# sideprotocol/plonky2-gpu

Hardware: AMD Instinct MI355X
Metric: NTTs/sec at 2^20 Goldilocks (higher is better)
Workload: dtype u64 (Goldilocks, integer modular)

## Files before the change

plonky2_gpu_amd/csrc/ntt_direct.hip:

```cpp

#include "ntt_kernels.h"

namespace plonky2_hip {
namespace nttk {

namespace {

#ifndef NTT_TAIL_GROUPED
#define NTT_TAIL_GROUPED 1
#endif
#ifndef DIRECT_DIAG_HOOKS
#define DIRECT_TILE_BARRIER() lds_barrier()
#define DIRECT_LOAD_TILE(t) (t)
#define DIRECT_STORE_TILE(t) (t)
#define DIRECT_DIAG_TAIL_FRONT_ON 0
#define DIRECT_DIAG_SAME_STORES_ON 0
#define DIRECT_NT_LOAD_COL false
#define DIRECT_NT_STORE_COL false
#define DIRECT_NT_LOAD_ROW false
#define DIRECT_NT_STORE_ROW false
#define DIRECT_TOUCH_STATE
#define DIRECT_TOUCH_COL(t_in_a)
#define DIRECT_TOUCH_ROW(t_in_a)
#endif

__device__ __forceinline__ uint64_t lds_ld(const unsigned char *lds, uint32_t off) { return *reinterpret_cast<const uint64_t *>(lds + off); }
__device__ __forceinline__ void lds_st(unsigned char *lds, uint32_t off, uint64_t v) { *reinterpret_cast<uint64_t *>(lds + off) = v; }
template <bool NT = false>
__device__ __forceinline__ uint64_t g_ld(const uint64_t *base, uint32_t byte_off) {
    const uint64_t *q = reinterpret_cast<const uint64_t *>(reinterpret_cast<const unsigned char *>(base) + byte_off);
    if constexpr (NT) return __builtin_nontemporal_load(q);
    return *q;
}
template <bool NT = false>
__device__ __forceinline__ void g_st(uint64_t *base, uint32_t byte_off, uint64_t v) {
    uint64_t *q = reinterpret_cast<uint64_t *>(reinterpret_cast<unsigned char *>(base) + byte_off);
    if constexpr (NT)
        __builtin_nontemporal_store(v, q);
    else
        *q = v;
}
constexpr bool NT_LOAD_COL = DIRECT_NT_LOAD_COL, NT_STORE_COL = DIRECT_NT_STORE_COL, NT_LOAD_ROW = DIRECT_NT_LOAD_ROW, NT_STORE_ROW = DIRECT_NT_STORE_ROW;

template <int LOGG>
struct ColGeom {
    static constexpr int G = 1 << LOGG, LOGC = 6 - LOGG, C = 1 << LOGC, LOGR = 8 + LOGG, R = 1 << LOGR;
    static constexpr uint32_t ROWB = C * 8;
    static constexpr uint32_t SA = 16 * ROWB + (G >= 4 ? ROWB : 0);
    static constexpr uint32_t XBYTES = 16 * G * SA;
    static constexpr uint32_t TWBYTES = 16 * G * 16 * 8;
    static constexpr uint32_t LDS_BYTES = XBYTES + TWBYTES;
    static constexpr uint32_t cu_entries(uint32_t gz) { return gz * (G > 1 ? G * 16 : 256); }
    static constexpr uint32_t t2z_entries(uint32_t gz) { return G > 1 ? gz * 16 * G : 0; }
    static constexpr uint32_t cs_entries(uint32_t gz) { return gz * C; }
    static constexpr uint32_t coset_bytes(uint32_t gz) { return (cu_entries(gz) + t2z_entries(gz) + cs_entries(gz)) * 8; }
};

static_assert(ColGeom<3>::LDS_BYTES <= 160 * 1024 && ColGeom<2>::LDS_BYTES <= 160 * 1024, "the exchange image and the tables must fit the 160 KiB of LDS of a gfx950 CU");

template <int LOGG, bool NATURAL, bool COSET = false, bool FINAL = false, bool REVIN = false>
__global__ __launch_bounds__(1024) __attribute__((amdgpu_waves_per_eu(4, 4))) void ntt_col_direct_kernel(const PassParams p, const uint32_t gx, const uint32_t gy, const uint32_t gz, const uint32_t per_b) {
    using GEO = ColGeom<LOGG>;
    constexpr int G = GEO::G, LOGC = GEO::LOGC, C = GEO::C, LOGR = GEO::LOGR;
    constexpr uint32_t ROWB = GEO::ROWB, SA = GEO::SA;
    extern __shared__ __attribute__((aligned(16))) unsigned char ldsb[];
    unsigned char *X = ldsb;
    unsigned char *TW = ldsb + GEO::XBYTES;
    unsigned char *CU = TW + GEO::TWBYTES, *T2Z = CU + GEO::cu_entries(gz) * 8, *CS = T2Z + GEO::t2z_entries(gz) * 8;

    const uint32_t tid = threadIdx.x, lane = tid & 63;
    const uint32_t wave = __builtin_amdgcn_readfirstlane(tid >> 6);
    const uint32_t g = lane >> LOGC, c = lane & (C - 1);

    const uint32_t W = gridDim.x;
    const uint32_t u = (W & 7) == 0 ? (blockIdx.x & 7) * (W >> 3) + (blockIdx.x >> 3) : blockIdx.x;
    const uint32_t P = gy * gz;
    uint32_t b0, bstep, p0, pstep;
    if (per_b) {
        if constexpr (COSET) b0 = u / per_b, p0 = u % per_b;
        else b0 = u % gx, p0 = u / gx;
        bstep = gx, pstep = per_b;
    } else {
        b0 = u, bstep = W, p0 = 0, pstep = 1;
    }
    const uint32_t np_local = p0 < P ? (P - p0 + pstep - 1) / pstep : 0;
    const uint32_t nb_local = b0 < gx ? (gx - b0 + bstep - 1) / bstep : 0;
    const uint32_t n_tiles = np_local * nb_local;
    if (n_tiles == 0) return;

    for (uint32_t e = tid; e < 16u * G * 16u; e += 1024) {
        const uint32_t w_ = e / (16 * G), g_ = (e / 16) % G, ka = e % 16;
        reinterpret_cast<uint64_t *>(TW)[e] = p.twh[(ka * (16 * g_ + w_)) << (12 - LOGR)];
    }
    uint64_t t2[G > 1 ? G : 1];
    if constexpr (!COSET)
        static_for<1, G>([&](auto K_) {
            constexpr int kb = decltype(K_)::value;
            t2[kb] = p.twh[(kb * wave) << (12 - 4 - LOGG)];
        });
    if constexpr (COSET) {
        auto cs_pow = [&](uint32_t z, uint64_t ex) { return gl::mul(p.cs_hi[z * p.cs_hi_len + (uint32_t)(ex >> 10)], p.cs_lo[z * 1024 + (uint32_t)(ex & 1023)]); };
        for (uint32_t e = tid; e < GEO::cu_entries(gz); e += 1024) {
            const uint32_t i = e & 15, mid = G > 1 ? 16 * ((e >> 4) % G) : (e >> 4) & 15, z = G > 1 ? e / (16 * G) : e >> 8;
            reinterpret_cast<uint64_t *>(CU)[e] = cs_pow(z, (uint64_t)p.in_m * (((uint32_t)i << (LOGR - 4)) + mid));
        }
        for (uint32_t e = tid; e < GEO::t2z_entries(gz); e += 1024) {
            const uint32_t kb = e % G, w_ = (e / G) & 15, z = e / (16 * G);
            reinterpret_cast<uint64_t *>(T2Z)[e] = gl::mul(p.twh[(kb * w_) << (12 - 4 - LOGG)], cs_pow(z, (uint64_t)p.in_m * w_));
        }
        for (uint32_t e = tid; e < GEO::cs_entries(gz); e += 1024)
            reinterpret_cast<uint64_t *>(CS)[e] = cs_pow(e / C, (uint64_t)b0 * C + (e % C));
    }

    const uint32_t tw_base = (wave * G + g) * 128;
    const uint32_t lane_x = wave * ROWB + c * 8;
    const uint32_t pw_base = 16 * g * SA + lane_x;
    const uint32_t pr_base = g * SA + lane_x;
    constexpr bool natural = NATURAL;
    auto opaque_lane = [&]() {
        uint32_t l = lane;
        asm volatile("" : "+v"(l));
        return l;
    };
    auto kab_of = [&](uint32_t l) { return G * wave + (l >> LOGC); };
    auto xr_base_of = [&](uint32_t l) { return kab_of(l) * SA + (l & (C - 1)) * 8; };
    auto ld_off_of = [&](uint32_t l) { return (uint32_t)(((l & (C - 1)) + (uint64_t)(16 * (l >> LOGC) + wave) * p.in_m) * 8); };
    const uint64_t out_c = p.out_c ? p.out_c : 1;
    auto st_off_of = [&](uint32_t l) {
        const uint32_t kab = kab_of(l);
        const uint32_t out_row_lane = natural ? kab : (brev_rt(kab & 15, 4) << (LOGR - 4)) | (brev_rt(kab >> 4, LOGG) << 4);
        return (uint32_t)(((l & (C - 1)) * out_c + (uint64_t)out_row_lane * p.out_m) * 8);
    };

    auto tile_of = [&](uint32_t t, uint32_t &b, uint32_t &a, uint32_t &z) {
        const uint32_t bi = t / np_local, pi = t - bi * np_local;
        b = b0 + bi * bstep;
        const uint32_t pp = p0 + pi * pstep;
        if constexpr (COSET) a = pp / gz, z = pp % gz;
        else a = pp % gy, z = pp / gy;
        if (p.sweep_down) a = gy - 1 - a;
    };

    uint64_t A[16];
    const uint32_t ld_step = (uint32_t)(((uint64_t)p.in_m << (LOGR - 4)) * 8);
    auto issue_loads = [&](uint32_t t) {
        uint32_t b, a, z;
        tile_of(DIRECT_LOAD_TILE(t), b, a, z);
        if constexpr (REVIN) {
            static_assert(!COSET && NATURAL, "the reversed-input pass is the first pass of a natural-order inverse transform");
            const uint64_t *base = p.src + (a * p.in_sa + z * p.in_sz);
            const uint32_t l = opaque_lane();
            const uint32_t L = b * C + (l & (C - 1)), m0 = 16 * (l >> LOGC) + wave;
            const uint32_t cols = (uint32_t)p.in_m;
            uint32_t off = L ? (((uint32_t)GEO::R - 1 - m0) * cols + (cols - L)) * 8 : (((uint32_t)GEO::R - m0) * cols) * 8;
            const bool wraps = L == 0 && m0 == 0;
            static_for<0, 16>([&](auto I_) {
                constexpr int i = decltype(I_)::value;
                if constexpr (i == 0) A[i] = g_ld<NT_LOAD_COL>(base, wraps ? 0u : off);
                else A[i] = g_ld<NT_LOAD_COL>(base, off);
                if constexpr (i < 15) off -= ld_step;
            });
            return;
        }
        const uint64_t *base = p.src + (a * p.in_sa + b * p.in_sb + z * p.in_sz);
        uint32_t off = ld_off_of(opaque_lane());
        static_for<0, 16>([&](auto I_) {
            constexpr int i = decltype(I_)::value;
            A[i] = g_ld<NT_LOAD_COL>(base, off);
            if constexpr (i < 15) off += ld_step;
        });
    };

    uint64_t B[16];
    uint64_t cc0 = 1, cstep = 1;
    constexpr bool kept_twiddles = !COSET && !FINAL;
    uint64_t cw[kept_twiddles ? 8 : 1], cstep8 = 1;
    uint32_t chain_b = 0xFFFFFFFFu;
    const uint32_t st_row = (uint32_t)(p.out_m * 8);

    uint64_t cc = 1;
    uint64_t *obase = p.dst;
    uint32_t so = 0;
    auto tail_begin = [&](uint32_t k) {
        uint32_t b, a, z;
        tile_of(k, b, a, z);
        if (!FINAL && b != chain_b) {
            chain_b = b;
            const uint32_t l = opaque_lane();
            const uint64_t L = (uint64_t)b * C + (l & (C - 1));
            cc0 = wpow(p, L * kab_of(l));
            if (p.chain_scale != 1) cc0 = gl::mul(cc0, p.chain_scale);
            cstep = wpow(p, L << (4 + LOGG));
            asm volatile("" : "+v"(cc0), "+v"(cstep));
            if constexpr (kept_twiddles) {
                cw[0] = cc0;
                static_for<1, 8>([&](auto J_) {
                    constexpr int j = decltype(J_)::value;
                    cw[j] = gl::mul(cw[j - 1], cstep);
                });
                const uint64_t s2 = gl::mul(cstep, cstep), s4 = gl::mul(s2, s2);
                cstep8 = gl::mul(s4, s4);
            }
        }
        if constexpr (DIRECT_DIAG_SAME_STORES_ON) tile_of(0, b, a, z);
        obase = p.dst + (a * p.out_sa + b * p.out_sb + (COSET ? brev_rt(z, p.rate_bits) : z) * p.out_sz);
        if constexpr (COSET) cc = gl::mul(cc0, lds_ld(CS, (z * C + (opaque_lane() & (C - 1))) * 8));
        else cc = cc0;
        so = st_off_of(opaque_lane());
    };
    auto tail_unit = [&](auto J_) {
        constexpr int j = decltype(J_)::value;
        constexpr int s3 = brev_c(j, 4);
        if constexpr (FINAL) {
            B[s3] = gl::canon(B[s3]);
        } else if constexpr (kept_twiddles) {
            if constexpr (j < 8) B[s3] = gl::mul(B[s3], cw[j]);
            else B[s3] = gl::mul(B[s3], gl::mul(cw[j - 8], cstep8));
        } else {
            B[s3] = gl::mul(B[s3], cc);
            if constexpr (j < 15) cc = gl::mul(cc, cstep);
        }
        const uint32_t row = natural ? (uint32_t)(j << (4 + LOGG)) : (uint32_t)s3;
        g_st<NT_STORE_COL>(obase, so + row * st_row, B[s3]);
        __builtin_amdgcn_sched_barrier(0);
    };
    auto tail_store = [&](auto J_) {
        constexpr int j = decltype(J_)::value;
        constexpr int s3 = brev_c(j, 4);
        const uint32_t row = natural ? (uint32_t)(j << (4 + LOGG)) : (uint32_t)s3;
        g_st<NT_STORE_COL>(obase, so + row * st_row, B[s3]);
        __builtin_amdgcn_sched_barrier(0);
    };
    auto tail_units = [&](auto LO_, auto HI_) {
        constexpr int LO = decltype(LO_)::value, HI = decltype(HI_)::value, N = HI - LO;
        if constexpr (NTT_TAIL_GROUPED && kept_twiddles && N >= 1 && N <= 8) {
            uint64_t tw[N];
            constexpr int N_HI = HI > 8 ? HI - (LO > 8 ? LO : 8) : 0;
            if constexpr (N_HI > 0)
                rare_group<N_HI>([&](auto I_, gl::rare_mask &f) { constexpr int j = (LO > 8 ? LO : 8) + decltype(I_)::value; tw[j - LO] = gl::mul_f(cw[j - 8], cstep8, f); },
                                 [&](auto I_, gl::rare_mask f) { constexpr int j = (LO > 8 ? LO : 8) + decltype(I_)::value; tw[j - LO] = gl::mul_fix(tw[j - LO], f); });
            rare_group<N>(
                [&](auto I_, gl::rare_mask &f) {
                    constexpr int j = LO + decltype(I_)::value, s3 = brev_c(j, 4);
                    if constexpr (j < 8) B[s3] = gl::mul_f(B[s3], cw[j], f);
                    else B[s3] = gl::mul_f(B[s3], tw[j - LO], f);
                },
                [&](auto I_, gl::rare_mask f) {
                    constexpr int s3 = brev_c(LO + decltype(I_)::value, 4);
                    B[s3] = gl::mul_fix(B[s3], f);
                });
            static_for<LO, HI>([&](auto J_) { tail_store(J_); });
        } else {
            static_for<LO, HI>([&](auto J_) { tail_unit(J_); });
        }
    };

    DIRECT_TOUCH_STATE
    auto first_rounds = [&](auto WITH_TAIL_, uint32_t t_in_a) {
        constexpr bool with_tail = decltype(WITH_TAIL_)::value;
        uint32_t zc = 0;
        if constexpr (COSET) {
            uint32_t b_, a_;
            tile_of(t_in_a, b_, a_, zc);
        }
        if constexpr (with_tail && DIRECT_DIAG_TAIL_FRONT_ON) tail_units(std::integral_constant<int, 0>{}, std::integral_constant<int, 16>{});
#define TAIL(lo, hi) do { if constexpr (with_tail && !DIRECT_DIAG_TAIL_FRONT_ON) tail_units(std::integral_constant<int, lo>{}, std::integral_constant<int, hi>{}); } while (0)
        TAIL(0, 4);
        if constexpr (COSET) {
            const uint32_t cu_base = (G > 1 ? (zc * G + (opaque_lane() >> LOGC)) * 16 : (zc * 16 + wave) * 16) * 8;
            mul_run<0, 16>(A, [](auto I_) { return decltype(I_)::value; }, [&](auto I_) { return lds_ld(CU, cu_base + decltype(I_)::value * 8); }, [](auto) {});
        }
        radix_dif_stage<4, 0, 3>(A);
        DIRECT_TOUCH_COL(t_in_a);
        TAIL(4, 6);
        radix_dif_stage<4, 0, 2>(A);
        TAIL(6, 8);
        radix_dif_stage<4, 0, 1>(A);
        TAIL(8, 10);
        radix_dif_stage<4, 0, 0>(A);
        TAIL(10, 12);
        mul_run<1, 16>(A, [](auto S_) { return decltype(S_)::value; }, [&](auto S_) { return lds_ld(TW, tw_base + brev_c(decltype(S_)::value, 4) * 8); },
                       [&](auto S_) {
                           constexpr int s = decltype(S_)::value;
                           if constexpr (s == 5) TAIL(12, 13);
                           if constexpr (s == 10) TAIL(13, 14);
                       });
        if constexpr (G > 1) {
            static_for<0, 16>([&](auto S_) {
                constexpr int s = decltype(S_)::value;
                constexpr int ka = brev_c(s, 4);
                lds_st(X, pw_base + ka * SA, A[s]);
            });
            tile_sync<64>();
            static_for<0, 16 / G>([&](auto J_) {
                constexpr int j = decltype(J_)::value;
                static_for<0, G>([&](auto GG_) {
                    constexpr int gg = decltype(GG_)::value;
                    A[j * G + gg] = lds_ld(X, pr_base + (16 * gg + G * j) * SA);
                });
            });
            tile_sync<64>();
            radix_dif_blocks<LOGG>(A);
            TAIL(14, 15);
            if constexpr (COSET)
                mul_run<0, 16>(A, [](auto E_) { return decltype(E_)::value; },
                               [&](auto E_) { return lds_ld(T2Z, ((zc * 16 + wave) * G + brev_c(decltype(E_)::value % G, LOGG)) * 8); }, [](auto) {});
            else
                mul_run<0, (G - 1) * (16 / G)>(A, [](auto K_) { return (decltype(K_)::value / (G - 1)) * G + 1 + decltype(K_)::value % (G - 1); },
                                               [&](auto K_) { return t2[brev_c(1 + decltype(K_)::value % (G - 1), LOGG)]; }, [](auto) {});
            static_for<0, 16 / G>([&](auto J_) {
                constexpr int j = decltype(J_)::value;
                static_for<0, G>([&](auto S_) {
                    constexpr int s2 = decltype(S_)::value;
                    constexpr int kb = brev_c(s2, LOGG);
                    lds_st(X, pr_base + (G * j + 16 * kb) * SA, A[j * G + s2]);
                });
            });
            TAIL(15, 16);
        } else {
            TAIL(14, 16);
            static_for<0, 16>([&](auto S_) {
                constexpr int s = decltype(S_)::value;
                constexpr int ka = brev_c(s, 4);
                lds_st(X, pr_base + ka * SA, A[s]);
            });
        }
#undef TAIL
    };

    lds_barrier();
    issue_loads(0);
    const uint32_t last = n_tiles - 1;
    first_rounds(std::false_type{}, 0);
    if (last > 0) issue_loads(1);
#pragma unroll 1
    for (uint32_t k = 0; k <= last; k++) {
        DIRECT_TILE_BARRIER();
        const uint32_t xr_base = xr_base_of(opaque_lane());
        static_for<0, 16>([&](auto WR_) {
            constexpr int wr = decltype(WR_)::value;
            B[wr] = lds_ld(X, xr_base + wr * ROWB);
        });
        DIRECT_TILE_BARRIER();
        radix_dif<4, 0>(B);
        tail_begin(k);
        if (k < last) {
            first_rounds(std::true_type{}, k + 1);
            if (k + 1 < last) issue_loads(k + 2);
        } else {
            tail_units(std::integral_constant<int, 0>{}, std::integral_constant<int, 16>{});
        }
    }
}

template <int LOGG, bool NATURAL, bool COSET = false, bool FINAL = false, bool REVIN = false>
hipError_t launch_col_direct_t(const PassParams &p, dim3 grid, hipStream_t stream) {
    using GEO = ColGeom<LOGG>;
    const uint32_t lds_bytes = GEO::LDS_BYTES + (COSET ? GEO::coset_bytes(grid.z) : 0);
    static DynamicLds attr;
    if (hipError_t e = allow_dynamic_lds(attr, reinterpret_cast<const void *>(&ntt_col_direct_kernel<LOGG, NATURAL, COSET, FINAL, REVIN>), lds_bytes); e != hipSuccess) return e;
    int dev = 0, cus = 256;
    if (hipGetDevice(&dev) == hipSuccess) (void)hipDeviceGetAttribute(&cus, hipDeviceAttributeMultiprocessorCount, dev);
    const uint64_t pairs = (uint64_t)grid.y * grid.z, total = pairs * grid.x;
    if (total == 0) return hipSuccess;
    if (total > 0xFFFFFFFFull) return hipErrorInvalidValue;
    uint32_t per_b = 0, wgs;
    if (grid.x <= (uint32_t)cus) {
        per_b = (uint32_t)cus / grid.x;
        if (per_b > pairs) per_b = (uint32_t)pairs;
        wgs = grid.x * per_b;
    } else {
        wgs = (uint32_t)cus;
    }
    if (COSET && per_b == 0) return hipErrorInvalidValue;
    hipLaunchKernelGGL((ntt_col_direct_kernel<LOGG, NATURAL, COSET, FINAL, REVIN>), dim3(wgs), dim3(1024), lds_bytes, stream, p, (uint32_t)grid.x, (uint32_t)grid.y, (uint32_t)grid.z, per_b);
    return hipGetLastError();
}


struct RowGeom {
    static constexpr uint32_t SQ = 136, SB = 544, SA = 8736;
    static constexpr uint32_t XBYTES = 16 * SA;
    static constexpr uint32_t TW1_STRIDE = 136, TW1_BYTES = 64 * TW1_STRIDE;
    static constexpr uint32_t TW2_STRIDE = 136, TW2_BYTES = 4 * TW2_STRIDE;
    static constexpr uint32_t LDS_BYTES = XBYTES + TW1_BYTES;
};

template <bool INVERSE>
__global__ __launch_bounds__(1024) __attribute__((amdgpu_waves_per_eu(4, 4))) void ntt_row_natural_direct_kernel(const PassParams p, const uint32_t gx, const uint32_t gy, const uint32_t gz) {
    using GEO = RowGeom;
    constexpr uint32_t SQ = GEO::SQ, SB = GEO::SB, SA = GEO::SA;
    extern __shared__ __attribute__((aligned(16))) unsigned char ldsb[];
    unsigned char *X = ldsb;
    unsigned char *TW1 = ldsb + GEO::XBYTES;

    const uint32_t tid = threadIdx.x, lane = tid & 63;
    const uint32_t wave = __builtin_amdgcn_readfirstlane(tid >> 6);

    const uint32_t W = gridDim.x;
    const uint32_t u = (W & 7) == 0 ? (blockIdx.x & 7) * (W >> 3) + (blockIdx.x >> 3) : blockIdx.x;
    const uint32_t total = gx * gy * gz;
    if (u >= total) return;
    const uint32_t n_tiles = (total - u + W - 1) / W;

    for (uint32_t e = tid; e < 64 * 16; e += 1024) {
        const uint32_t l = e >> 4, ka = e & 15;
        *reinterpret_cast<uint64_t *>(TW1 + l * GEO::TW1_STRIDE + ka * 8) = p.twh[(ka * l) << 2];
    }

    const uint32_t q = lane & 3, hi4 = lane >> 2;
    const uint32_t tw1_base = lane * GEO::TW1_STRIDE;
    const uint32_t pw_base = hi4 * SB + q * SQ + wave * 8;
    const uint32_t pr_base = hi4 * SA + q * SQ + wave * 8;
    auto opaque_lane = [&]() {
        uint32_t l = lane;
        asm volatile("" : "+v"(l));
        return l;
    };

    auto tile_of = [&](uint32_t t, uint32_t &b, uint32_t &a, uint32_t &z) {
        const uint32_t id = u + t * W;
        b = id % gx;
        const uint32_t r = id / gx;
        a = r % gy;
        z = r / gy;
        if (p.sweep_down) a = gy - 1 - a;
    };

    uint64_t A[16];
    auto issue_loads = [&](uint32_t t) {
        uint32_t b, a, z;
        tile_of(DIRECT_LOAD_TILE(t), b, a, z);
        const uint32_t row = (b * 16 + wave + p.row_shift) & (p.t_limit - 1);
        const uint64_t *base = p.src + (a * p.in_sa + z * p.in_sz + (uint64_t)row * p.in_t);
        const uint32_t off = opaque_lane() * 8;
        static_for<0, 16>([&](auto I_) {
            constexpr int i = decltype(I_)::value;
            A[i] = g_ld<NT_LOAD_ROW>(base, off + i * 512);
        });
    };

    uint64_t B[16];
    const uint32_t kbhi = wave >> 2, kalo = wave & 3;
    uint64_t *obase = p.dst;
    uint32_t o_lane = 0;
    const uint32_t n_mask = (1u << p.log_n) - 1;
    auto tail_begin = [&](uint32_t k) {
        uint32_t b, a, z;
        tile_of(DIRECT_STORE_TILE(k), b, a, z);
        obase = p.dst + (a * p.out_sa + z * p.out_sz);
        const uint32_t l = opaque_lane();
        const uint32_t r = l & 15, ka = 4 * (l >> 4) + kalo;
        const uint32_t k1 = (b * 16 + r + p.row_shift) & (p.t_limit - 1);
        o_lane = k1 + (uint32_t)p.out_m * (ka + 64 * kbhi);
    };
    auto tail_unit = [&](auto J_) {
        constexpr int s = decltype(J_)::value;
        constexpr int kblo = s >> 2, kc = brev_c(s & 3, 2);
// ... 212 lines not shown
            const uint32_t kbhi = l & 3, base = (l >> 2) * 32 + kbhi * 2048;
            static_for<0, 16>([&](auto R_) {
                constexpr int r = decltype(R_)::value;
                B[r] = lds_ld(X, base + (r >> 2) * 512 + (((uint32_t)(r & 3) ^ kbhi) * 8));
            });
        }
        tile_sync<64>();
        radix_dif_blocks<2>(B);
        {
            const uint32_t l = opaque_lane();
            const uint32_t ka = l >> 2, kbhi = l & 3;
            const uint32_t pa = brev_rt(ka, 4), sw = pa >> 2;
            const uint32_t base = (pa * 64 + brev_rt(kbhi, 2) * 4) * 8;
            static_for<0, 16>([&](auto R_) {
                constexpr int r = decltype(R_)::value;
                constexpr uint32_t kblo = r >> 2, s2 = r & 3;
                lds_st(X, base + brev_c(kblo, 2) * 128 + ((s2 ^ sw) * 8), gl::canon(B[r]));
            });
        }
        tile_sync<64>();
        {
            const uint32_t l = opaque_lane();
            uint64_t *obase = p.dst + row_ptr(k, true);
            static_for<0, 16>([&](auto R_) {
                constexpr int r = decltype(R_)::value;
                const uint32_t slot = r * 64 + (l & ~3u) + ((l & 3) ^ (uint32_t)(r >> 2));
                const uint64_t v = lds_ld(X, slot * 8);
                g_st(obase, l * 8 + r * 512, v);
            });
        }
        tile_sync<64>();
        __builtin_amdgcn_sched_barrier(0);
        if (more) issue_loads_other_half(k + 1);
        __builtin_amdgcn_sched_barrier(0);
    };

    lds_barrier();
    if (n_rows == 0) return;
    issue_loads(0);
    issue_loads_other_half(0);
    first_round();
    if (n_rows > 1) issue_loads(1);
#pragma unroll 1
    for (uint32_t k = 0; k < n_rows; k++) {
        rest_of_row(k, k + 1 < n_rows);
        if (k + 1 < n_rows) {
            first_round();
            if (k + 2 < n_rows) issue_loads(k + 2);
        }
    }
}

template <bool HALVES = false>
hipError_t launch_row_inplace_direct_t(const PassParams &p, dim3 grid, hipStream_t stream) {
    constexpr uint32_t lds_bytes = HALVES ? RowInplaceGeom::LDS_BYTES_HALVES : RowInplaceGeom::LDS_BYTES;
    static DynamicLds attr;
    if (hipError_t e = allow_dynamic_lds(attr, reinterpret_cast<const void *>(&ntt_row_inplace_direct_kernel<HALVES>), lds_bytes); e != hipSuccess) return e;
    int dev = 0, cus = 256;
    if (hipGetDevice(&dev) == hipSuccess) (void)hipDeviceGetAttribute(&cus, hipDeviceAttributeMultiprocessorCount, dev);
    const uint64_t rows_total = (uint64_t)p.t_limit * grid.y * grid.z * (HALVES ? 2 : 1);
    if (rows_total == 0) return hipSuccess;
    if (rows_total > 0xFFFFFFFFull) return hipErrorInvalidValue;
    const uint64_t need = (rows_total + 15) / 16;
    const uint32_t wgs = (uint32_t)(need < (uint64_t)cus ? need : (uint64_t)cus);
    hipLaunchKernelGGL(ntt_row_inplace_direct_kernel<HALVES>, dim3(wgs), dim3(1024), lds_bytes, stream, p, (uint32_t)rows_total, p.t_limit, (uint32_t)grid.y);
    return hipGetLastError();
}

}

bool col_direct_coset_ok(int logg, dim3 grid) {
    int dev = 0, cus = 256;
    if (hipGetDevice(&dev) == hipSuccess) (void)hipDeviceGetAttribute(&cus, hipDeviceAttributeMultiprocessorCount, dev);
    if (grid.x > (uint32_t)cus || grid.z == 0) return false;
    const uint32_t limit = device_lds_limit();
    switch (logg) {
        case 0: return ColGeom<0>::LDS_BYTES + ColGeom<0>::coset_bytes(grid.z) <= limit;
        case 1: return ColGeom<1>::LDS_BYTES + ColGeom<1>::coset_bytes(grid.z) <= limit;
        case 2: return ColGeom<2>::LDS_BYTES + ColGeom<2>::coset_bytes(grid.z) <= limit;
        default: return false;
    }
}

hipError_t launch_col_direct(int logg, const PassParams &p, dim3 grid, hipStream_t stream) {
    const bool nat = p.flags & F_NATURAL;
    if (p.flags & F_COSET) {
        if (nat || !col_direct_coset_ok(logg, grid)) return hipErrorInvalidValue;
        switch (logg) {
            case 0: return launch_col_direct_t<0, false, true>(p, grid, stream);
            case 1: return launch_col_direct_t<1, false, true>(p, grid, stream);
            case 2: return launch_col_direct_t<2, false, true>(p, grid, stream);
            default: return hipErrorInvalidValue;
        }
    }
    switch (logg) {
        case 0: return nat ? launch_col_direct_t<0, true>(p, grid, stream) : launch_col_direct_t<0, false>(p, grid, stream);
        case 1: return nat ? launch_col_direct_t<1, true>(p, grid, stream) : launch_col_direct_t<1, false>(p, grid, stream);
        case 2: return nat ? launch_col_direct_t<2, true>(p, grid, stream) : launch_col_direct_t<2, false>(p, grid, stream);
        case 3: return nat ? launch_col_direct_t<3, true>(p, grid, stream) : launch_col_direct_t<3, false>(p, grid, stream);
        default: return hipErrorInvalidValue;
    }
}


hipError_t launch_col_direct_reversed_input(const PassParams &p, dim3 grid, hipStream_t stream) {
    if (!(p.flags & F_NATURAL) || (p.flags & F_COSET) || p.in_t != 1 || p.in_m != (1u << 11) || p.in_sb != 8) return hipErrorInvalidValue;
    return launch_col_direct_t<3, true, false, false, true>(p, grid, stream);
}

hipError_t launch_col_direct_final(const PassParams &p, dim3 grid, hipStream_t stream) {
    if (!(p.flags & F_NATURAL) || (p.flags & F_COSET)) return hipErrorInvalidValue;
    return launch_col_direct_t<3, true, false, true>(p, grid, stream);
}

hipError_t launch_row_inplace_direct(const PassParams &p, dim3 grid, hipStream_t stream) { return launch_row_inplace_direct_t<false>(p, grid, stream); }
hipError_t launch_row_inplace_direct_2048(const PassParams &p, dim3 grid, hipStream_t stream) { return launch_row_inplace_direct_t<true>(p, grid, stream); }

hipError_t launch_row_natural_direct(const PassParams &p, dim3 grid, hipStream_t stream) {
    return (p.flags & F_INVERSE) ? launch_row_natural_direct_t<true>(p, grid, stream) : launch_row_natural_direct_t<false>(p, grid, stream);
}

}
}
```

plonky2_gpu_amd/csrc/ntt_kernels.h:

```cpp
#pragma once
#include <atomic>
#include <hip/hip_runtime.h>
#include <stdint.h>

#include <type_traits>

#include "gl_field.h"

namespace plonky2_hip {
namespace nttk {

enum : uint32_t { F_LOAD_ROWS = 1, F_STORE_ROWS = 2, F_NATURAL = 4, F_INVERSE = 8, F_COSET = 16,
                  F_WIDE = 32,
                  F_RAW_OUT = 64,
                  F_FINAL_COL = 128 };

struct PassParams {
    const uint64_t *src;
    uint64_t *dst;
    const uint64_t *twl;
    const uint64_t *twh;
    const uint64_t *cs_hi;
    const uint64_t *cs_lo;
    uint64_t in_sa, in_sb, in_sz, in_t, in_m;
// ... 192 lines not shown
    constexpr auto KQ = [](int kblo, int q) { return (39 * q * (4 * KBHI + kblo)) % 192; };
    constexpr auto NEGQ = [](int kblo, int q) { return (39 * q * (4 * KBHI + kblo)) % 192 >= 96; };
    {
        gl::rare_mask fm[12];
        static_for<0, 12>([&](auto I_) {
            constexpr int i = decltype(I_)::value, kblo = i / 3, q = 1 + i % 3, KK = KQ(kblo, q) % 96;
            v[4 * kblo + q] = gl::mul_pow2_f<KK>(v[4 * kblo + q], fm[i]);
        });
        __builtin_amdgcn_sched_barrier(RARE_FENCE_MASK);
        gl::rare_mask any = 0;
        static_for<0, 12>([&](auto I_) { any |= fm[decltype(I_)::value]; });
        if (GL_RARE_ANY(any))
            static_for<0, 12>([&](auto I_) {
                constexpr int i = decltype(I_)::value, kblo = i / 3, q = 1 + i % 3, KK = KQ(kblo, q) % 96;
                v[4 * kblo + q] = gl::mul_pow2_fix<KK>(v[4 * kblo + q], fm[i]);
            });
    }
    auto bfly = [&](auto CNEG_, auto I0_, auto I1_, gl::rare_mask &f0, gl::rare_mask &f1) {
        constexpr bool cneg = decltype(CNEG_)::value;
        constexpr int i0 = decltype(I0_)::value, i1 = decltype(I1_)::value;
        if constexpr (cneg) gl::bfly_f<false>(v[i0], v[i1], v[i1], v[i0], f1, f0);
        else gl::bfly_f<false>(v[i0], v[i1], v[i0], v[i1], f0, f1);
    };
    auto fix = [&](auto IS_SUM_, auto SHIFT_, auto I_, gl::rare_mask f, gl::rare_mask fshift) {
        constexpr bool is_sum = decltype(IS_SUM_)::value;
        constexpr int shift = decltype(SHIFT_)::value, i = decltype(I_)::value;
        if constexpr (shift == 0) {
            v[i] = is_sum ? gl::add_fix(v[i], f) : gl::sub_fix(v[i], f);
        } else {
            v[i] = gl::mul_pow2_fix<shift>(v[i], fshift);
            const uint64_t c = gl::masked_const<gl::eps_times_pow2(shift)>(f);
            v[i] = is_sum ? gl::add(v[i], c) : gl::sub(v[i], c);
        }
    };
    using std::integral_constant;
    using std::bool_constant;
    {
        gl::rare_mask f0[8], f1[8], fm[4];
        static_for<0, 4>([&](auto B_) {
            constexpr int kblo = decltype(B_)::value, b = 4 * kblo;
            bfly(bool_constant<NEGQ(kblo, 2)>{}, integral_constant<int, b>{}, integral_constant<int, b + 2>{}, f0[2 * kblo], f1[2 * kblo]);
            bfly(bool_constant<NEGQ(kblo, 1) != NEGQ(kblo, 3)>{}, integral_constant<int, b + 1>{}, integral_constant<int, b + 3>{}, f0[2 * kblo + 1], f1[2 * kblo + 1]);
        });
        static_for<0, 4>([&](auto B_) {
            constexpr int kblo = decltype(B_)::value;
            v[4 * kblo + 3] = gl::mul_pow2_f<48>(v[4 * kblo + 3], fm[kblo]);
        });
        __builtin_amdgcn_sched_barrier(RARE_FENCE_MASK);
        gl::rare_mask any = 0;
        static_for<0, 8>([&](auto I_) { any |= f0[decltype(I_)::value] | f1[decltype(I_)::value]; });
        static_for<0, 4>([&](auto I_) { any |= fm[decltype(I_)::value]; });
        if (GL_RARE_ANY(any))
            static_for<0, 4>([&](auto B_) {
                constexpr int kblo = decltype(B_)::value, b = 4 * kblo;
                constexpr bool na = NEGQ(kblo, 2), nb = NEGQ(kblo, 1) != NEGQ(kblo, 3);
                fix(bool_constant<!na>{}, integral_constant<int, 0>{}, integral_constant<int, b>{}, f0[2 * kblo], 0);
                fix(bool_constant<na>{}, integral_constant<int, 0>{}, integral_constant<int, b + 2>{}, f1[2 * kblo], 0);
                fix(bool_constant<!nb>{}, integral_constant<int, 0>{}, integral_constant<int, b + 1>{}, f0[2 * kblo + 1], 0);
                fix(bool_constant<nb>{}, integral_constant<int, 48>{}, integral_constant<int, b + 3>{}, f1[2 * kblo + 1], fm[kblo]);
            });
    }
    {
        gl::rare_mask f0[8], f1[8];
        static_for<0, 4>([&](auto B_) {
            constexpr int kblo = decltype(B_)::value, b = 4 * kblo;
            bfly(bool_constant<NEGQ(kblo, 1)>{}, integral_constant<int, b>{}, integral_constant<int, b + 1>{}, f0[2 * kblo], f1[2 * kblo]);
            bfly(bool_constant<NEGQ(kblo, 1)>{}, integral_constant<int, b + 2>{}, integral_constant<int, b + 3>{}, f0[2 * kblo + 1], f1[2 * kblo + 1]);
        });
        __builtin_amdgcn_sched_barrier(RARE_FENCE_MASK);
        gl::rare_mask any = 0;
        static_for<0, 8>([&](auto I_) { any |= f0[decltype(I_)::value] | f1[decltype(I_)::value]; });
        if (GL_RARE_ANY(any))
            static_for<0, 4>([&](auto B_) {
                constexpr int kblo = decltype(B_)::value, b = 4 * kblo;
                constexpr bool n1 = NEGQ(kblo, 1);
                fix(bool_constant<!n1>{}, integral_constant<int, 0>{}, integral_constant<int, b>{}, f0[2 * kblo], 0);
                fix(bool_constant<n1>{}, integral_constant<int, 0>{}, integral_constant<int, b + 1>{}, f1[2 * kblo], 0);
                fix(bool_constant<!n1>{}, integral_constant<int, 0>{}, integral_constant<int, b + 2>{}, f0[2 * kblo + 1], 0);
                fix(bool_constant<n1>{}, integral_constant<int, 0>{}, integral_constant<int, b + 3>{}, f1[2 * kblo + 1], 0);
            });
    }
}

template <int NT_>
__device__ __forceinline__ void tile_sync() {
    if constexpr (NT_ == 64) {
        __builtin_amdgcn_fence(__ATOMIC_ACQ_REL, "wavefront");
        __builtin_amdgcn_wave_barrier();
    } else {
        __syncthreads();
    }
}

__device__ __forceinline__ void lds_barrier() { asm volatile("s_waitcnt lgkmcnt(0)\n\ts_barrier" ::: "memory"); }


struct DynamicLds {
    std::atomic<uint8_t> set[64] = {};
};
inline uint32_t device_lds_limit() {
    int dev = 0, bytes = 0;
    if (hipGetDevice(&dev) != hipSuccess || hipDeviceGetAttribute(&bytes, hipDeviceAttributeMaxSharedMemoryPerBlock, dev) != hipSuccess || bytes <= 0)
        return 64 * 1024;
    return (uint32_t)bytes;
}
inline hipError_t allow_dynamic_lds(DynamicLds &st, const void *fn, uint32_t lds_bytes) {
    int dev = 0;
    hipError_t e = hipGetDevice(&dev);
    if (e != hipSuccess) return e;
    std::atomic<uint8_t> &slot = st.set[dev & 63];
    if (slot.load(std::memory_order_acquire)) return hipSuccess;
    const uint32_t limit = device_lds_limit();
    e = hipFuncSetAttribute(fn, hipFuncAttributeMaxDynamicSharedMemorySize, (int)(lds_bytes > limit ? lds_bytes : limit));
    if (e != hipSuccess) return e;
    slot.store(1, std::memory_order_release);
    return hipSuccess;
}

hipError_t launch_col_direct(int logg, const PassParams &p, dim3 grid, hipStream_t stream);
hipError_t launch_col_direct_reversed_input(const PassParams &p, dim3 grid, hipStream_t stream);
hipError_t launch_col_direct_final(const PassParams &p, dim3 grid, hipStream_t stream);
bool col_direct_coset_ok(int logg, dim3 grid);
hipError_t launch_row_natural_direct(const PassParams &p, dim3 grid, hipStream_t stream);
hipError_t launch_row_inplace_direct(const PassParams &p, dim3 grid, hipStream_t stream);
hipError_t launch_row_inplace_direct_2048(const PassParams &p, dim3 grid, hipStream_t stream);

}
}
```

Measured before the change: 131,800.

## Split column-pass LDS exchange into two halves and keep upper twiddles in LDS

For the LOGG=2 column pass, the exchange image is halved and written in two phases. Waves are staggered so half read the image while the other half write their second half. Eight-plus of the sixteen per-column twiddles are precomputed into an LDS region instead of being derived with an extra multiply, which cuts register pressure and per-element multiplies. It adds barriers and LDS traffic, and includes optional (default-off) shift-twiddle radix and half-load variants.

```diff
diff --git a/plonky2_gpu_amd/csrc/ntt_direct.hip b/plonky2_gpu_amd/csrc/ntt_direct.hip
--- a/plonky2_gpu_amd/csrc/ntt_direct.hip
+++ b/plonky2_gpu_amd/csrc/ntt_direct.hip
@@ -1,4 +1,5 @@
 
+#include "knobs.h"
 #include "ntt_kernels.h"
 
 namespace plonky2_hip {
@@ -8,6 +9,18 @@
 
 #ifndef NTT_TAIL_GROUPED
 #define NTT_TAIL_GROUPED 1
+#endif
+#ifndef NTT_COL_RESIDENT_TWIDDLES
+#define NTT_COL_RESIDENT_TWIDDLES 1
+#endif
+#ifndef NTT_COL_SHIFT_TWIDDLE
+#define NTT_COL_SHIFT_TWIDDLE 0
+#endif
+#ifndef NTT_COL_LOAD_HALVES
+#define NTT_COL_LOAD_HALVES 0
+#endif
+#ifndef NTT_COL_CW_REGS
+#define NTT_COL_CW_REGS 6
 #endif
 #ifndef DIRECT_DIAG_HOOKS
 #define DIRECT_TILE_BARRIER() lds_barrier()
@@ -50,6 +63,10 @@
     static constexpr uint32_t XBYTES = 16 * G * SA;
     static constexpr uint32_t TWBYTES = 16 * G * 16 * 8;
     static constexpr uint32_t LDS_BYTES = XBYTES + TWBYTES;
+    static constexpr uint32_t XBYTES_SPLIT = 8 * G * SA;
+    static constexpr int CW_REGS = NTT_COL_CW_REGS;
+    static constexpr uint32_t CW_STRIDE = 1024 * 8, CWBYTES = (16 - CW_REGS) * CW_STRIDE;
+    static constexpr uint32_t LDS_BYTES_SPLIT = XBYTES_SPLIT + TWBYTES + CWBYTES;
     static constexpr uint32_t cu_entries(uint32_t gz) { return gz * (G > 1 ? G * 16 : 256); }
     static constexpr uint32_t t2z_entries(uint32_t gz) { return G > 1 ? gz * 16 * G : 0; }
     static constexpr uint32_t cs_entries(uint32_t gz) { return gz * C; }
@@ -57,15 +74,28 @@
 };
 
 static_assert(ColGeom<3>::LDS_BYTES <= 160 * 1024 && ColGeom<2>::LDS_BYTES <= 160 * 1024, "the exchange image and the tables must fit the 160 KiB of LDS of a gfx950 CU");
-
-template <int LOGG, bool NATURAL, bool COSET = false, bool FINAL = false, bool REVIN = false>
+static_assert(ColGeom<2>::CW_REGS >= 1 && ColGeom<2>::CW_REGS <= 8, "the kept twiddles");
+static_assert(ColGeom<2>::LDS_BYTES_SPLIT == 69632 + 8192 + (16 - ColGeom<2>::CW_REGS) * 8192 && ColGeom<2>::LDS_BYTES_SPLIT <= 160 * 1024, "two-phase image, TW and the resident twiddles");
+
+template <int LOGG, bool COSET, bool FINAL, bool REVIN, bool PREVIOUS>
+struct ColForm {
+    static constexpr bool tuned = LOGG == 2 && !COSET && !FINAL && !REVIN && !PREVIOUS;
+    static constexpr bool SPLIT = tuned && NTT_COL_RESIDENT_TWIDDLES;
+    static constexpr bool SHIFT2 = tuned && NTT_COL_SHIFT_TWIDDLE;
+    static constexpr uint32_t LDS_BYTES = SPLIT ? ColGeom<LOGG>::LDS_BYTES_SPLIT : ColGeom<LOGG>::LDS_BYTES;
+};
+
+template <int LOGG, bool NATURAL, bool COSET = false, bool FINAL = false, bool REVIN = false, bool PREVIOUS = false>
 __global__ __launch_bounds__(1024) __attribute__((amdgpu_waves_per_eu(4, 4))) void ntt_col_direct_kernel(const PassParams p, const uint32_t gx, const uint32_t gy, const uint32_t gz, const uint32_t per_b) {
     using GEO = ColGeom<LOGG>;
+    using FORM = ColForm<LOGG, COSET, FINAL, REVIN, PREVIOUS>;
+    constexpr bool SPLIT = FORM::SPLIT, SHIFT2 = FORM::SHIFT2;
     constexpr int G = GEO::G, LOGC = GEO::LOGC, C = GEO::C, LOGR = GEO::LOGR;
     constexpr uint32_t ROWB = GEO::ROWB, SA = GEO::SA;
     extern __shared__ __attribute__((aligned(16))) unsigned char ldsb[];
     unsigned char *X = ldsb;
-    unsigned char *TW = ldsb + GEO::XBYTES;
+    unsigned char *TW = ldsb + (SPLIT ? GEO::XBYTES_SPLIT : GEO::XBYTES);
+    unsigned char *CW = TW + GEO::TWBYTES;
     unsigned char *CU = TW + GEO::TWBYTES, *T2Z = CU + GEO::cu_entries(gz) * 8, *CS = T2Z + GEO::t2z_entries(gz) * 8;
 
     const uint32_t tid = threadIdx.x, lane = tid & 63;
@@ -93,7 +123,7 @@
         reinterpret_cast<uint64_t *>(TW)[e] = p.twh[(ka * (16 * g_ + w_)) << (12 - LOGR)];
     }
     uint64_t t2[G > 1 ? G : 1];
-    if constexpr (!COSET)
+    if constexpr (!COSET && !SHIFT2)
         static_for<1, G>([&](auto K_) {
             constexpr int kb = decltype(K_)::value;
             t2[kb] = p.twh[(kb * wave) << (12 - 4 - LOGG)];
@@ -114,7 +144,7 @@
 
     const uint32_t tw_base = (wave * G + g) * 128;
     const uint32_t lane_x = wave * ROWB + c * 8;
-    const uint32_t pw_base = 16 * g * SA + lane_x;
+    const uint32_t pw_base = (SPLIT ? 8 : 16) * g * SA + lane_x;
     const uint32_t pr_base = g * SA + lane_x;
     constexpr bool natural = NATURAL;
     auto opaque_lane = [&]() {
@@ -123,7 +153,7 @@
         return l;
     };
     auto kab_of = [&](uint32_t l) { return G * wave + (l >> LOGC); };
-    auto xr_base_of = [&](uint32_t l) { return kab_of(l) * SA + (l & (C - 1)) * 8; };
+    auto xr_base_of = [&](uint32_t l) { return (SPLIT ? kab_of(l) & (8 * G - 1) : kab_of(l)) * SA + (l & (C - 1)) * 8; };
     auto ld_off_of = [&](uint32_t l) { return (uint32_t)(((l & (C - 1)) + (uint64_t)(16 * (l >> LOGC) + wave) * p.in_m) * 8); };
     const uint64_t out_c = p.out_c ? p.out_c : 1;
     auto st_off_of = [&](uint32_t l) {
@@ -143,10 +173,12 @@
 
     uint64_t A[16];
     const uint32_t ld_step = (uint32_t)(((uint64_t)p.in_m << (LOGR - 4)) * 8);
-    auto issue_loads = [&](uint32_t t) {
+    auto issue_loads_part = [&](uint32_t t, auto LO_, auto HI_) {
+        constexpr int LO = decltype(LO_)::value, HI = decltype(HI_)::value;
         uint32_t b, a, z;
         tile_of(DIRECT_LOAD_TILE(t), b, a, z);
         if constexpr (REVIN) {
+            static_assert(LO == 0 && HI == 16, "the reversed-input pass loads whole tiles");
             static_assert(!COSET && NATURAL, "the reversed-input pass is the first pass of a natural-order inverse transform");
             const uint64_t *base = p.src + (a * p.in_sa + z * p.in_sz);
             const uint32_t l = opaque_lane();
@@ -163,18 +195,22 @@
             return;
         }
         const uint64_t *base = p.src + (a * p.in_sa + b * p.in_sb + z * p.in_sz);
-        uint32_t off = ld_off_of(opaque_lane());
-        static_for<0, 16>([&](auto I_) {
+        uint32_t off = ld_off_of(opaque_lane()) + LO * ld_step;
+        static_for<LO, HI>([&](auto I_) {
             constexpr int i = decltype(I_)::value;
             A[i] = g_ld<NT_LOAD_COL>(base, off);
-            if constexpr (i < 15) off += ld_step;
-        });
-    };
+            if constexpr (i < HI - 1) off += ld_step;
+        });
+    };
+    auto issue_loads = [&](uint32_t t) { issue_loads_part(t, std::integral_constant<int, 0>{}, std::integral_constant<int, 16>{}); };
+    uint64_t N[16];
 
     uint64_t B[16];
     uint64_t cc0 = 1, cstep = 1;
     constexpr bool kept_twiddles = !COSET && !FINAL;
-    uint64_t cw[kept_twiddles ? 8 : 1], cstep8 = 1;
+    constexpr int KEPT = SPLIT ? GEO::CW_REGS : 8;
+    uint64_t cw[kept_twiddles ? KEPT : 1], cstep8 = 1;
+    auto cw_off = [&](int j) { return (wave * 64 + opaque_lane()) * 8 + (uint32_t)(j - KEPT) * GEO::CW_STRIDE; };
     uint32_t chain_b = 0xFFFFFFFFu;
     const uint32_t st_row = (uint32_t)(p.out_m * 8);
 
@@ -194,12 +230,20 @@
             asm volatile("" : "+v"(cc0), "+v"(cstep));
             if constexpr (kept_twiddles) {
                 cw[0] = cc0;
-                static_for<1, 8>([&](auto J_) {
+                static_for<1, KEPT>([&](auto J_) {
                     constexpr int j = decltype(J_)::value;
                     cw[j] = gl::mul(cw[j - 1], cstep);
                 });
-                const uint64_t s2 = gl::mul(cstep, cstep), s4 = gl::mul(s2, s2);
-                cstep8 = gl::mul(s4, s4);
+                if constexpr (SPLIT) {
+                    uint64_t t = cw[KEPT - 1];
+                    static_for<KEPT, 16>([&](auto J_) {
+                        t = gl::mul(t, cstep);
+                        lds_st(CW, cw_off(decltype(J_)::value), t);
+                    });
+                } else {
+                    const uint64_t s2 = gl::mul(cstep, cstep), s4 = gl::mul(s2, s2);
+                    cstep8 = gl::mul(s4, s4);
+                }
             }
         }
         if constexpr (DIRECT_DIAG_SAME_STORES_ON) tile_of(0, b, a, z);
@@ -214,7 +258,8 @@
         if constexpr (FINAL) {
             B[s3] = gl::canon(B[s3]);
         } else if constexpr (kept_twiddles) {
-            if constexpr (j < 8) B[s3] = gl::mul(B[s3], cw[j]);
+            if constexpr (j < KEPT) B[s3] = gl::mul(B[s3], cw[j]);
+            else if constexpr (SPLIT) B[s3] = gl::mul(B[s3], lds_ld(CW, cw_off(j)));
             else B[s3] = gl::mul(B[s3], gl::mul(cw[j - 8], cstep8));
         } else {
             B[s3] = gl::mul(B[s3], cc);
@@ -235,14 +280,16 @@
         constexpr int LO = decltype(LO_)::value, HI = decltype(HI_)::value, N = HI - LO;
         if constexpr (NTT_TAIL_GROUPED && kept_twiddles && N >= 1 && N <= 8) {
             uint64_t tw[N];
-            constexpr int N_HI = HI > 8 ? HI - (LO > 8 ? LO : 8) : 0;
-            if constexpr (N_HI > 0)
+            constexpr int N_HI = HI > KEPT ? HI - (LO > KEPT ? LO : KEPT) : 0;
+            if constexpr (N_HI > 0 && SPLIT)
+                static_for<(LO > KEPT ? LO : KEPT), HI>([&](auto J_) { constexpr int j = decltype(J_)::value; tw[j - LO] = lds_ld(CW, cw_off(j)); });
+            else if constexpr (N_HI > 0)
                 rare_group<N_HI>([&](auto I_, gl::rare_mask &f) { constexpr int j = (LO > 8 ? LO : 8) + decltype(I_)::value; tw[j - LO] = gl::mul_f(cw[j - 8], cstep8, f); },
                                  [&](auto I_, gl::rare_mask f) { constexpr int j = (LO > 8 ? LO : 8) + decltype(I_)::value; tw[j - LO] = gl::mul_fix(tw[j - LO], f); });
             rare_group<N>(
                 [&](auto I_, gl::rare_mask &f) {
                     constexpr int j = LO + decltype(I_)::value, s3 = brev_c(j, 4);
-                    if constexpr (j < 8) B[s3] = gl::mul_f(B[s3], cw[j], f);
+                    if constexpr (j < KEPT) B[s3] = gl::mul_f(B[s3], cw[j], f);
                     else B[s3] = gl::mul_f(B[s3], tw[j - LO], f);
                 },
                 [&](auto I_, gl::rare_mask f) {
@@ -285,7 +332,39 @@
                            if constexpr (s == 5) TAIL(12, 13);
                            if constexpr (s == 10) TAIL(13, 14);
                        });
-        if constexpr (G > 1) {
+        if constexpr (SPLIT) {
+            static_for<0, 2>([&](auto H_) {
+                constexpr int h = decltype(H_)::value;
+                static_for<0, 16>([&](auto S_) {
+                    constexpr int s = decltype(S_)::value;
+                    constexpr int ka = brev_c(s, 4);
+                    if constexpr ((ka >> 3) == h) lds_st(X, pw_base + (ka & 7) * SA, A[s]);
+                });
+                tile_sync<64>();
+                static_for<2 * h, 2 * h + 2>([&](auto J_) {
+                    constexpr int j = decltype(J_)::value;
+                    static_for<0, G>([&](auto GG_) {
+                        constexpr int gg = decltype(GG_)::value;
+                        N[j * G + gg] = lds_ld(X, pr_base + (8 * gg + G * (j - 2 * h)) * SA);
+                    });
+                });
+                tile_sync<64>();
+            });
+            radix_dif_blocks<LOGG>(N);
+            TAIL(14, 15);
+            if constexpr (!SHIFT2)
+                mul_run<0, (G - 1) * (16 / G)>(N, [](auto K_) { return (decltype(K_)::value / (G - 1)) * G + 1 + decltype(K_)::value % (G - 1); },
+                                               [&](auto K_) { return t2[brev_c(1 + decltype(K_)::value % (G - 1), LOGG)]; }, [](auto) {});
+            static_for<0, 16 / G>([&](auto J_) {
+                constexpr int j = decltype(J_)::value;
+                static_for<0, G>([&](auto S_) {
+                    constexpr int s2 = decltype(S_)::value;
+                    constexpr int kb = brev_c(s2, LOGG);
+                    if constexpr (kb < G / 2) lds_st(X, pr_base + (G * j + 16 * kb) * SA, N[j * G + s2]);
+                });
+            });
+            TAIL(15, 16);
+        } else if constexpr (G > 1) {
             static_for<0, 16>([&](auto S_) {
                 constexpr int s = decltype(S_)::value;
                 constexpr int ka = brev_c(s, 4);
@@ -305,7 +384,7 @@
             if constexpr (COSET)
                 mul_run<0, 16>(A, [](auto E_) { return decltype(E_)::value; },
                                [&](auto E_) { return lds_ld(T2Z, ((zc * 16 + wave) * G + brev_c(decltype(E_)::value % G, LOGG)) * 8); }, [](auto) {});
-            else
+            else if constexpr (!SHIFT2)
                 mul_run<0, (G - 1) * (16 / G)>(A, [](auto K_) { return (decltype(K_)::value / (G - 1)) * G + 1 + decltype(K_)::value % (G - 1); },
                                                [&](auto K_) { return t2[brev_c(1 + decltype(K_)::value % (G - 1), LOGG)]; }, [](auto) {});
             static_for<0, 16 / G>([&](auto J_) {
@@ -332,33 +411,81 @@
     issue_loads(0);
     const uint32_t last = n_tiles - 1;
     first_rounds(std::false_type{}, 0);
-    if (last > 0) issue_loads(1);
-#pragma unroll 1
-    for (uint32_t k = 0; k <= last; k++) {
-        DIRECT_TILE_BARRIER();
+    using std::integral_constant;
+    constexpr bool LOAD_HALVES = SPLIT && NTT_COL_LOAD_HALVES;
+    if constexpr (LOAD_HALVES) {
+        if (last > 0) issue_loads_part(1, integral_constant<int, 0>{}, integral_constant<int, 8>{});
+    } else {
+        if (last > 0) issue_loads(1);
+    }
+    auto read_image = [&]() {
         const uint32_t xr_base = xr_base_of(opaque_lane());
         static_for<0, 16>([&](auto WR_) {
             constexpr int wr = decltype(WR_)::value;
             B[wr] = lds_ld(X, xr_base + wr * ROWB);
         });
+    };
+#pragma unroll 1
+    for (uint32_t k = 0; k <= last; k++) {
+        auto finish_tile = [&]() {
+            if constexpr (SHIFT2) {
+                const uint32_t kb = wave >> 2;
+                if (kb == 0) radix_dif<4, 0>(B);
+                else if (kb == 1) shift_twiddles_radix16<1>(B);
+                else if (kb == 2) shift_twiddles_radix16<2>(B);
+                else shift_twiddles_radix16<3>(B);
+            } else {
+                radix_dif<4, 0>(B);
+            }
+            tail_begin(k);
+        };
         DIRECT_TILE_BARRIER();
-        radix_dif<4, 0>(B);
-        tail_begin(k);
+        if constexpr (SPLIT) {
+            auto phase2 = [&]() {
+                DIRECT_TILE_BARRIER();
+                static_for<0, 16 / G>([&](auto J_) {
+                    constexpr int j = decltype(J_)::value;
+                    static_for<0, G>([&](auto S_) {
+                        constexpr int s2 = decltype(S_)::value;
+                        constexpr int kb = brev_c(s2, LOGG);
+                        if constexpr (kb >= G / 2) lds_st(X, pr_base + (G * j + 16 * (kb - G / 2)) * SA, N[j * G + s2]);
+                    });
+                });
+                if constexpr (LOAD_HALVES)
+                    if (k < last) issue_loads_part(k + 1, integral_constant<int, 8>{}, integral_constant<int, 16>{});
+                DIRECT_TILE_BARRIER();
+            };
+            if (wave < 8) {
+                read_image();
+                phase2();
+            } else {
+                phase2();
+                read_image();
+            }
+        } else {
+            read_image();
+        }
+        DIRECT_TILE_BARRIER();
+        finish_tile();
         if (k < last) {
             first_rounds(std::true_type{}, k + 1);
-            if (k + 1 < last) issue_loads(k + 2);
+            if constexpr (LOAD_HALVES) {
+                if (k + 1 < last) issue_loads_part(k + 2, integral_constant<int, 0>{}, integral_constant<int, 8>{});
+            } else {
+                if (k + 1 < last) issue_loads(k + 2);
+            }
         } else {
             tail_units(std::integral_constant<int, 0>{}, std::integral_constant<int, 16>{});
         }
     }
 }
 
-template <int LOGG, bool NATURAL, bool COSET = false, bool FINAL = false, bool REVIN = false>
+template <int LOGG, bool NATURAL, bool COSET = false, bool FINAL = false, bool REVIN = false, bool PREVIOUS = false>
 hipError_t launch_col_direct_t(const PassParams &p, dim3 grid, hipStream_t stream) {
     using GEO = ColGeom<LOGG>;
-    const uint32_t lds_bytes = GEO::LDS_BYTES + (COSET ? GEO::coset_bytes(grid.z) : 0);
+    const uint32_t lds_bytes = ColForm<LOGG, COSET, FINAL, REVIN, PREVIOUS>::LDS_BYTES + (COSET ? GEO::coset_bytes(grid.z) : 0);
     static DynamicLds attr;
-    if (hipError_t e = allow_dynamic_lds(attr, reinterpret_cast<const void *>(&ntt_col_direct_kernel<LOGG, NATURAL, COSET, FINAL, REVIN>), lds_bytes); e != hipSuccess) return e;
+    if (hipError_t e = allow_dynamic_lds(attr, reinterpret_cast<const void *>(&ntt_col_direct_kernel<LOGG, NATURAL, COSET, FINAL, REVIN, PREVIOUS>), lds_bytes); e != hipSuccess) return e;
     int dev = 0, cus = 256;
     if (hipGetDevice(&dev) == hipSuccess) (void)hipDeviceGetAttribute(&cus, hipDeviceAttributeMultiprocessorCount, dev);
     const uint64_t pairs = (uint64_t)grid.y * grid.z, total = pairs * grid.x;
@@ -373,7 +500,7 @@
         wgs = (uint32_t)cus;
     }
     if (COSET && per_b == 0) return hipErrorInvalidValue;
-    hipLaunchKernelGGL((ntt_col_direct_kernel<LOGG, NATURAL, COSET, FINAL, REVIN>), dim3(wgs), dim3(1024), lds_bytes, stream, p, (uint32_t)grid.x, (uint32_t)grid.y, (uint32_t)grid.z, per_b);
+    hipLaunchKernelGGL((ntt_col_direct_kernel<LOGG, NATURAL, COSET, FINAL, REVIN, PREVIOUS>), dim3(wgs), dim3(1024), lds_bytes, stream, p, (uint32_t)grid.x, (uint32_t)grid.y, (uint32_t)grid.z, per_b);
     return hipGetLastError();
 }
 
@@ -752,6 +879,13 @@
     }
 }
 
+#ifdef PLONKY2_DEBUG_KNOBS
+static bool previous_col_pass() {
+    const char *e = PLONKY2_KNOB("PLONKY2_NTT_COL_SPLIT");
+    return e && e[0] == '0';
+}
+#endif
+
 hipError_t launch_col_direct(int logg, const PassParams &p, dim3 grid, hipStream_t stream) {
     const bool nat = p.flags & F_NATURAL;
     if (p.flags & F_COSET) {
@@ -766,7 +900,11 @@
     switch (logg) {
         case 0: return nat ? launch_col_direct_t<0, true>(p, grid, stream) : launch_col_direct_t<0, false>(p, grid, stream);
         case 1: return nat ? launch_col_direct_t<1, true>(p, grid, stream) : launch_col_direct_t<1, false>(p, grid, stream);
-        case 2: return nat ? launch_col_direct_t<2, true>(p, grid, stream) : launch_col_direct_t<2, false>(p, grid, stream);
+        case 2:
+#ifdef PLONKY2_DEBUG_KNOBS
+            if (previous_col_pass()) return nat ? launch_col_direct_t<2, true, false, false, false, true>(p, grid, stream) : launch_col_direct_t<2, false, false, false, false, true>(p, grid, stream);
+#endif
+            return nat ? launch_col_direct_t<2, true>(p, grid, stream) : launch_col_direct_t<2, false>(p, grid, stream);
         case 3: return nat ? launch_col_direct_t<3, true>(p, grid, stream) : launch_col_direct_t<3, false>(p, grid, stream);
         default: return hipErrorInvalidValue;
     }
diff --git a/plonky2_gpu_amd/csrc/ntt_kernels.h b/plonky2_gpu_amd/csrc/ntt_kernels.h
--- a/plonky2_gpu_amd/csrc/ntt_kernels.h
+++ b/plonky2_gpu_amd/csrc/ntt_kernels.h
@@ -298,6 +298,78 @@
     }
 }
 
+constexpr bool col_shift_sign(int KB, int before_stage, int slot) {
+    bool n[16] = {};
+    for (int w = 0; w < 16; w++) n[w] = (39 * KB * w) % 192 >= 96;
+    for (int s = 3; s > before_stage; s--) {
+        const int half = 1 << s;
+        for (int bb = 0; bb < 8; bb++) {
+            const int i0 = (bb / half) * 2 * half + (bb % half), i1 = i0 + half;
+            const int K = (39 * (bb % half) * (32 >> s)) % 192;
+            const bool n0 = n[i0], n1 = n[i1];
+            if (n0 == n1) n[i1] = false;
+            else n[i0] = false, n[i1] = n0 != (K >= 96);
+        }
+    }
+    return n[slot];
+}
+constexpr bool col_shift_signs_absorbed(int KB) {
+    for (int i = 0; i < 16; i++)
+        if (col_shift_sign(KB, -1, i)) return false;
+    return true;
+}
+template <int KB, int s>
+__device__ __forceinline__ void radix16_signed_stage(uint64_t (&v)[16]) {
+    constexpr int half = 1 << s;
+    gl::rare_mask f0[8], f1[8], fm[8];
+    static_for<0, 8>([&](auto B_) {
+        constexpr int bb = decltype(B_)::value;
+        constexpr int i0 = (bb / half) * 2 * half + (bb % half), i1 = i0 + half;
+        constexpr int K = (39 * (bb % half) * (32 >> s)) % 192;
+        constexpr bool n0 = col_shift_sign(KB, s, i0), n1 = col_shift_sign(KB, s, i1);
+        if constexpr (n0 == n1) gl::bfly_f<(n0 != (K >= 96))>(v[i0], v[i1], v[i0], v[i1], f0[bb], f1[bb]);
+        else gl::bfly_f<n0>(v[i0], v[i1], v[i1], v[i0], f1[bb], f0[bb]);
+    });
+    static_for<0, 8>([&](auto B_) {
+        constexpr int bb = decltype(B_)::value;
+        constexpr int i1 = (bb / half) * 2 * half + (bb % half) + half;
+        constexpr int KK = (39 * (bb % half) * (32 >> s)) % 96;
+        if constexpr (s > 0) v[i1] = gl::mul_pow2_f<KK>(v[i1], fm[bb]);
+        else fm[bb] = 0;
+    });
+    __builtin_amdgcn_sched_barrier(RARE_FENCE_MASK);
+    gl::rare_mask any = 0;
+    static_for<0, 8>([&](auto B_) { constexpr int b = decltype(B_)::value; any |= f0[b] | f1[b] | fm[b]; });
+    if (GL_RARE_ANY(any))
+        static_for<0, 8>([&](auto B_) {
+            constexpr int bb = decltype(B_)::value;
+            constexpr int i0 = (bb / half) * 2 * half + (bb % half), i1 = i0 + half;
+            constexpr int KK = (39 * (bb % half) * (32 >> s)) % 96;
+            constexpr bool same = col_shift_sign(KB, s, i0) == col_shift_sign(KB, s, i1);
+            v[i0] = same ? gl::add_fix(v[i0], f0[bb]) : gl::sub_fix(v[i0], f0[bb]);
+            if constexpr (s > 0) {
+                v[i1] = gl::mul_pow2_fix<KK>(v[i1], fm[bb]);
+                const uint64_t c = gl::masked_const<gl::eps_times_pow2(KK)>(f1[bb]);
+                v[i1] = same ? gl::sub(v[i1], c) : gl::add(v[i1], c);
+            } else {
+                v[i1] = same ? gl::sub_fix(v[i1], f1[bb]) : gl::add_fix(v[i1], f1[bb]);
+            }
+        });
+}
+template <int KB>
+__device__ __forceinline__ void shift_twiddles_radix16(uint64_t (&v)[16]) {
+    static_assert(KB >= 1 && KB <= 3 && col_shift_signs_absorbed(KB), "every sign must be absorbed by the order of a subtraction");
+    static_for<0, 2>([&](auto G_) {
+        constexpr int w0 = 1 + 8 * decltype(G_)::value, n = w0 == 1 ? 8 : 7;
+        rare_group<n>([&](auto I_, gl::rare_mask &f) { constexpr int w = w0 + decltype(I_)::value; v[w] = gl::mul_pow2_f<(39 * KB * w) % 96>(v[w], f); },
+                      [&](auto I_, gl::rare_mask f) { constexpr int w = w0 + decltype(I_)::value; v[w] = gl::mul_pow2_fix<(39 * KB * w) % 96>(v[w], f); });
+    });
+    radix16_signed_stage<KB, 3>(v);
+    radix16_signed_stage<KB, 2>(v);
+    radix16_signed_stage<KB, 1>(v);
+    radix16_signed_stage<KB, 0>(v);
+}
+
 template <int NT_>
 __device__ __forceinline__ void tile_sync() {
     if constexpr (NT_ == 64) {
```

After: 132,200 (median of 6 runs). No clear change (+0.3%).
